# bbuchfink/diamond

Measured on AMD Instinct MI355X. Metric: GCUPS + aligned queries/s, blastp --fast, 10000 queries vs 1000000-seq DB (seed stage + banded SW extension), higher is better.
Workload: dtype int16

## Files before the change

### diamond_amd/csrc/seed_api.hip

```cpp
#include <hip/hip_runtime.h>
#include <algorithm>
#include <cstdlib>
#include <cmath>
#include <cstdio>
#include <cstring>
#include <string>
#include <sys/mman.h>
#include <thread>
#include <vector>
#include <chrono>
#include "ctx.h"
#include "seed_core.h"
#include "seed_kernels.h"

using namespace dmnd;

enum { SEED_CLASSES_LONG_DEFAULT = 1 };

static_assert(sizeof(dmnd_seed_params) == sizeof(SeedParams), "dmnd_seed_params must mirror dmnd::SeedParams");
static_assert(sizeof(dmnd_seed_hit) == 24, "dmnd_seed_hit layout");

extern "C" int dmnd_seed_params_fast(dmnd_seed_params* p, int threads)
{
	if (!p || threads < 1) return fail(DMND_E_ARG, "dmnd_seed_params_fast: bad argument");
// ... 281 lines not shown
			float ms = 0;
			if (hipEventElapsedTime(&ms, x.a, x.b) == hipSuccess) *x.into += ms;
			(void)hipEventDestroy(x.a); (void)hipEventDestroy(x.b);
		}
		spans.clear();
	}
};

}

struct SeedSizes {
	uint64_t slots, bm_words, bm1_words;
	uint32_t bm1_k3;
	int SB, slot_shift;
	bool fused, reuse;
	size_t bm_total;
};

static SeedSizes seed_sizes(const dmnd_ctx* c, const SeedParams& sp, int64_t nq_pos)
{
	SeedSizes z;
	const int S = sp.n_shapes;
	const uint64_t slots_x8 = (uint64_t)(tuning().seed_slots_x8 ? tuning().seed_slots_x8 : (seed_stream_can_fuse(sp) ? 32 : 16));
	z.slots = 1024;
	while (z.slots * 8 < (uint64_t)nq_pos * slots_x8) z.slots <<= 1;
	while (z.slots > ((uint64_t)1 << 31) && z.slots / 2 >= (uint64_t)nq_pos + (uint64_t)nq_pos / 4) z.slots >>= 1;

	uint64_t bm_words = 1 << 15;
	while (bm_words * 32 < (uint64_t)nq_pos * 16 && bm_words < ((uint64_t)1 << 22)) bm_words <<= 1;
	int bm1_log2 = 24;
	if (nq_pos > ((int64_t)1 << 24))
		while (bm1_log2 < 27 && ((uint64_t)1 << bm1_log2) < (uint64_t)nq_pos * 4) ++bm1_log2;
	uint64_t bm1_words = ((uint64_t)1 << bm1_log2) / 32;
	if (bm1_words > bm_words) bm1_words = bm_words;
	uint32_t bm1_k3 = 0;
	const bool long_seeds = !seed_stream_can_fuse(sp);
	if (long_seeds && bm1_log2 == 24 && bm_words >= 3 * bm1_words / 2) {
		bm1_words = 3 * bm1_words / 2;
		bm1_k3 = (uint64_t)nq_pos * 4 <= bm1_words * 32 ? 1u : 0u;
	}
	if (!long_seeds && bm1_log2 == 24 && bm_words >= 2 * bm1_words) { bm1_words *= 2; bm1_k3 = 1u; }
	bool fused = seed_stream_can_fuse(sp);
	if (const char* e = getenv("DMND_SEED_FUSED")) fused = fused && atoi(e) != 0;
	z.slot_shift = 4;
	const size_t set_bytes = (z.slots << z.slot_shift) + 2 * (size_t)nq_pos * sizeof(uint32_t) + (size_t)(bm_words + bm1_words) * sizeof(uint32_t);
	const bool reuse = c->reuse_query_index && set_bytes * (size_t)S <= ((size_t)64 << 30) && !getenv("DMND_SEED_MATCHED_CAP");
	const int SB = (fused && !reuse) ? 1 : S;
	const size_t bm_total = (size_t)SB * (bm_words + bm1_words) * sizeof(uint32_t);
	z.bm_words = bm_words; z.bm1_words = bm1_words; z.bm1_k3 = bm1_k3;
	z.fused = fused; z.reuse = reuse; z.SB = SB; z.bm_total = bm_total;
	return z;
}

static int seed_reserve(dmnd_ctx* c, const SeedParams& sp, const SeedSizes& z, int64_t nq_pos, int64_t q_end, int64_t q_block_len, bool generous)
{
	if (int rc = c->seed_bitmap.ensure(z.bm_total)) return rc;
	{
		const size_t held = c->qid_of.cap;
		if (int rc = c->qid_of.ensure((size_t)q_end * sizeof(uint32_t))) return rc;
		if (c->qid_of.cap != held) c->qid_of_version = ~(uint64_t)0;
	}
	if (int rc = c->mask_time.ensure((size_t)q_block_len + 256)) return rc;
	if (int rc = c->seed_keys.ensure((size_t)z.SB * (z.slots << z.slot_shift))) return rc;
	if (int rc = c->seed_need.ensure((size_t)(z.slots / 32 + SEED_NEED_FOLD_WORDS) * sizeof(uint32_t))) return rc;
	if (int rc = c->seed_next.ensure((size_t)seed_build_work_words(nq_pos) * sizeof(uint32_t))) return rc;
	if (int rc = c->seed_qlist.ensure((size_t)z.SB * nq_pos * sizeof(uint32_t))) return rc;
	if (int rc = c->seed_qkeys.ensure((size_t)nq_pos * sizeof(uint32_t))) return rc;
	if (!generous) return DMND_OK;
	const int64_t m_cap = std::max<int64_t>((int64_t)1 << 22, 4 * nq_pos);
	if (int rc = c->matched_slot.ensure((size_t)m_cap * sizeof(uint32_t))) return rc;
	if (int rc = c->matched_loc.ensure((size_t)m_cap * sizeof(int64_t))) return rc;
	if (int rc = c->seed_hits.ensure(((size_t)1 << 20) * sizeof(dmnd_seed_hit))) return rc;
	if (int rc = c->seed_deferred.ensure(((size_t)1 << 18) * sizeof(SeedDeferred))) return rc;
	if (z.fused) {
		if (int rc = c->seed_survivors.ensure(((size_t)1 << 20) * sizeof(SeedSurvivor))) return rc;
		if (int rc = c->seed_qfold.ensure((size_t)(q_block_len + 1) / 2 + 64)) return rc;
	}
	else {
		if (int rc = c->seed_survivors.ensure(((size_t)1 << 20) * sizeof(SeedSurvivor))) return rc;
		if (int rc = c->seed_scored.ensure(((size_t)1 << 20) * sizeof(SeedScored))) return rc;
	}
	return DMND_OK;
}

int dmnd_seed_query_ids(dmnd_ctx* c)
{
	const std::vector<int64_t>& ql = c->limits[DMND_QUERY];
	if (ql.size() < 2) return DMND_OK;
	const size_t bytes = (size_t)ql.back() * sizeof(uint32_t);
	if (c->qid_of_version == c->query_limits_version && c->qid_of.cap >= bytes) return DMND_OK;
	if (int rc = c->qid_of.ensure(bytes)) return rc;
	HIP_TRY(launch_seed_qid(c->d_limits[DMND_QUERY].as<int64_t>(), (int64_t)ql.size() - 1, c->qid_of.as<uint32_t>(), c->stream));
	c->qid_of_version = c->query_limits_version;
	return DMND_OK;
}

extern "C" int dmnd_seed_reserve(dmnd_ctx* c, const dmnd_seed_params* params, int64_t query_block_len)
{
	if (!c || !params || query_block_len <= 512) return fail(DMND_E_ARG, "dmnd_seed_reserve: bad argument");
	SeedParams sp;
	std::memcpy(&sp, params, sizeof(sp));
	if (sp.n_shapes < 1 || sp.n_shapes > SEED_MAX_SHAPES) return fail(DMND_E_ARG, "dmnd_seed_reserve: unsupported seed configuration");
	HIP_TRY(hipSetDevice(c->device));
	const int64_t nq_pos = query_block_len - 512;
	return seed_reserve(c, sp, seed_sizes(c, sp, nq_pos), nq_pos, query_block_len - 256, query_block_len, true);
}

namespace {

struct SeedHooks {
	bool trace;
	int chain, tiled, slices;
	int classes_long;
	uint64_t slices_budget;
	int64_t slices_min_letters;
	uint32_t slice_words;
	int64_t matched_cap, survivor_cap, hit_cap, deferred_cap;
	int64_t sort_cap, readback_bytes;
};
SeedHooks seed_hooks()
{
	auto num = [](const char* name, long long unset) { const char* e = getenv(name); return e ? atoll(e) : unset; };
	auto forced = [](const char* name) { const char* e = getenv(name); return e ? (atoi(e) != 0 ? 1 : 0) : -1; };
	auto cap = [](const char* name) { const char* e = getenv(name); return e ? std::max<int64_t>(1, atoll(e)) : (int64_t)0; };
	SeedHooks h;
	h.trace = getenv("DMND_TRACE") != nullptr;
	h.chain = forced("DMND_SEED_CHAIN"); h.tiled = forced("DMND_SEED_TILED"); h.slices = forced("DMND_SEED_SLICES");
	{ const char* e = getenv("DMND_SEED_CLASSES_LONG"); h.classes_long = e ? atoi(e) : -1; }
	h.slices_budget = (uint64_t)std::max<long long>(0, num("DMND_SEED_SLICES_BUDGET_MB", tuning().seed_slices_budget_mb)) << 20;
	h.slices_min_letters = num("DMND_SEED_SLICES_MIN_LETTERS", tuning().seed_slices_min_letters);
	h.slice_words = (uint32_t)std::min<long long>(SEED_SLICE_MAX_WORDS, std::max<long long>(64, num("DMND_SEED_SLICE_WORDS", SEED_SLICE_MAX_WORDS)));
	h.matched_cap = cap("DMND_SEED_MATCHED_CAP"); h.survivor_cap = cap("DMND_SEED_SURVIVOR_CAP");
	h.hit_cap = cap("DMND_SEED_HIT_CAP"); h.deferred_cap = cap("DMND_SEED_DEFERRED_CAP");
	const int64_t sort_cap = cap("DMND_SEED_SORT_CAP");
	h.sort_cap = std::min<int64_t>(sort_cap ? sort_cap : tuning().seed_sort_cap, (int64_t)1 << 24);
	h.readback_bytes = std::min<int64_t>(std::max<int64_t>(0, num("DMND_SEED_READBACK_BYTES", tuning().seed_readback_bytes)), (int64_t)1 << 30);
	return h;
}
int64_t cap_or(int64_t hook, int64_t computed) { return hook ? hook : computed; }

struct PostState {
	unsigned long long hits_seen = 0;
	bool hits_fresh = false;
	unsigned long long def_max = 0;
};
struct FusedHits { int64_t cap = 0, bound = 0; };

struct SeedRun {
	dmnd_ctx* c;
	SeedHooks hooks;
	SeedParams sp;
	hipStream_t st;
	int64_t q_begin = 0, q_end = 0, t_begin = 0, t_end = 0, nq_pos = 0, n_targets = 0;
	int S = 0;
	SeedSizes z;
	int slot_bits = 0, bm_log2 = 0;
	size_t slot_bytes = 0;
	bool nibble_shapes = true, classes_long = false;
	int classes = 0;
	bool mlr_on = false, lin_on = false, phases = false;
	bool index_ready = false;
	std::string signature;
	int64_t tiled_from = 0;
	SeedRefUse ref_use = SEED_REF_NONE;
	int slice_bits = -1;
	int64_t ref_windows = 0;
	std::vector<unsigned long long> counts;
	std::vector<int64_t> m_off;
	bool pristine = true;
	Timer tm;
	char path[128] = "host";
	unsigned long long n_pairs = 0;
	std::chrono::steady_clock::time_point lap_t0 = std::chrono::steady_clock::now();

	SeedRun(dmnd_ctx* ctx, const SeedHooks& h) : c(ctx), hooks(h), st(ctx->stream), tm(ctx->stream) {}
	int check_blocks();
	int geometry();
	int prepare();
	int ref_cache();
	int fused();
	int fused_stage2(SeedArgs a, int sid, unsigned long long n, unsigned long long ns, FusedHits& fh, PostState& ps);
	int after_post(const SeedArgs& a, int sid, int64_t n_matched, int64_t def_cap, PostState& ps);
	SeedArgs chain_args(const SeedChain& ch, int64_t def_cap, int sid) const;
	int chain(ChainResume& res);
	int phase1(const ChainResume& res);
	int count_pairs();
	int phase2(const ChainResume& res);
	int pair_filter(SeedArgs& a, int sid);
	int sort_hits();
	void trace_summary() const;

	void lap(const char* what) const
	{
		if (hooks.trace) std::fprintf(stderr, "dmnd_seed_search %8.2f ms  %s\n", std::chrono::duration<double, std::milli>(std::chrono::steady_clock::now() - lap_t0).count(), what);
	}
	unsigned long long* ctr() const { return c->counters.as<unsigned long long>(); }

	SeedArgs args_for(int sid, int64_t matched_cap, int64_t matched_off) const
	{
		const int own = sid % z.SB;
		SeedArgs a;
		a.params = sp;
		a.qdata = c->block[DMND_QUERY].as<int8_t>(); a.tdata = c->block[DMND_TARGET].as<int8_t>();
		a.qseed = c->soft_valid[DMND_QUERY] ? c->soft[DMND_QUERY].as<int8_t>() : a.qdata;
		a.tseed = (c->soft_valid[DMND_TARGET] && sp.seed_encoding == SEED_SPACED) ? c->soft[DMND_TARGET].as<int8_t>() : a.tdata;
		a.qlimits = c->d_limits[DMND_QUERY].as<int64_t>();
		a.q_begin = q_begin; a.q_end = q_end; a.t_begin = t_begin; a.t_end = t_end;
		a.qid_of = c->qid_of.as<uint32_t>(); a.mask_time = c->mask_time.as<uint8_t>();
		a.tlimits = c->d_limits[DMND_TARGET].as<int64_t>(); a.n_targets = n_targets;
		a.qwin = mlr_on ? c->seed_qwin.as<SeedQueryWindow>() : nullptr;
		a.lin_first = lin_on ? c->seed_lin_first.as<int64_t>() : nullptr;
		a.slots = reinterpret_cast<SeedSlot*>(c->seed_keys.as<char>() + (size_t)own * slot_bytes);
		a.slot_shift = z.slot_shift;
		a.qlist = c->seed_qlist.as<uint32_t>() + (size_t)own * nq_pos;
		a.slot_mask = z.slots - 1;
		a.classes = classes;
		a.slot_bits = slot_bits;
		a.bm1_hmask = bm1_hmask_of(slot_bits, classes);
		a.bitmap_log2 = bm_log2;
		a.phase_ticks = phases ? ctr() + S + 8 : nullptr;
		a.tclass = classes ? c->seed_tclass.as<uint16_t>() : nullptr; a.tclass_stride = (seed_code_groups(t_begin, t_end) + 3) & ~(int64_t)3;
		a.tcodes = classes ? c->seed_tcodes.as<uint64_t>() : nullptr; a.tflags = classes ? c->seed_tflags.as<uint32_t>() : nullptr; a.tplanes = classes ? c->seed_tplanes.as<uint64_t>() : nullptr;
		a.bitmap = c->seed_bitmap.as<uint32_t>() + (size_t)own * (z.bm_words + z.bm1_words);
		a.bitmap1 = a.bitmap + z.bm_words;
		a.bitmap1_words = (uint32_t)z.bm1_words; a.bitmap1_k3 = z.bm1_k3;
		a.matched_slot = c->matched_slot.as<uint32_t>() + matched_off;
		a.matched_loc = c->matched_loc.as<int64_t>() + matched_off;
		a.matched_count = ctr() + sid;
		a.matched_cap = matched_cap;
		a.deferred = nullptr; a.deferred_count = ctr() + S + 1; a.deferred_cap = 0;
// ... 43 lines not shown
		return fail(DMND_E_ARG, "dmnd_seed_search: unsupported seed configuration");
	if (sp.reduction_size > 20) return fail(DMND_E_ARG, "dmnd_seed_search: more than 20 reduced letter classes");
	for (int l = 0; l < 32; ++l)
		if (!((sp.reduction[l] >= 0 && sp.reduction[l] < sp.reduction_size) || sp.reduction[l] == L_MASK))
			return fail(DMND_E_ARG, "dmnd_seed_search: reduction map entry outside [0, reduction_size) and not the mask letter");
	for (int i = 0; i < sp.n_shapes; ++i) {
		if (sp.shape_len[i] < 1 || sp.shape_len[i] > 32 || sp.shape_weight[i] < 1 || sp.shape_weight[i] > 19 || sp.shape_weight[i] > sp.shape_len[i])
			return fail(DMND_E_ARG, "dmnd_seed_search: bad shape (length 1..32, weight 1..19)");
		uint32_t mask = 0;
		for (int k = 0; k < sp.shape_weight[i]; ++k) {
			if (sp.shape_pos[i][k] < 0 || sp.shape_pos[i][k] >= sp.shape_len[i]) return fail(DMND_E_ARG, "dmnd_seed_search: shape position outside the shape");
			mask |= 1u << sp.shape_pos[i][k];
		}
		if (mask != sp.shape_mask[i]) return fail(DMND_E_ARG, "dmnd_seed_search: shape mask and positions disagree");
	}
	if (sp.seed_encoding != SEED_SPACED && sp.seed_encoding != SEED_HASHED) return fail(DMND_E_ARG, "dmnd_seed_search: unknown seed encoding");
	if (sp.seed_encoding == SEED_HASHED) {
		if (sp.index_chunks != 1 || sp.reduction_size > 16) return fail(DMND_E_ARG, "dmnd_seed_search: the query-indexed mode runs with one index chunk and a 4-bit reduction");
		for (int i = 0; i < sp.n_shapes; ++i)
			if (sp.shape_len[i] > 16) return fail(DMND_E_ARG, "dmnd_seed_search: query-indexed mode with a shape longer than 16 letters");
	}
	return DMND_OK;
}

int SeedRun::check_blocks()
{
	const std::vector<int64_t>& ql = c->limits[DMND_QUERY];
	const std::vector<int64_t>& tl = c->limits[DMND_TARGET];
	mlr_on = c->min_length_ratio > 0.0;
	c->seed_qwin_n = 0;
	if (mlr_on) {
		if (c->query_contexts != 1 || sp.query_translated) return fail(DMND_E_ARG, "dmnd_seed_search: a minimum length ratio is not supported for translated searches");
		if (!lengths_non_increasing(ql.data(), (int64_t)ql.size() - 1)) return fail(DMND_E_ARG, "dmnd_seed_search: with a minimum length ratio the query block must be length-sorted (dmnd_length_sort_order)");
		if (!lengths_non_increasing(tl.data(), (int64_t)tl.size() - 1)) return fail(DMND_E_ARG, "dmnd_seed_search: with a minimum length ratio the reference block must be length-sorted (dmnd_length_sort_order)");
	}
	lin_on = c->linsearch;
	if (lin_on) {
		for (int i = 0; i < sp.n_shapes; ++i)
			if (!lin_shape_weight_ok(sp.shape_weight[i])) return fail(DMND_E_ARG, "dmnd_seed_search: Linearization is only supported for seed shapes of weight >= 10.");
		if (mlr_on) return fail(DMND_E_ARG, "dmnd_seed_search: the linearised search together with a minimum length ratio is not supported (dmnd_set_linsearch, dmnd_set_min_length_ratio)");
		if (c->lin_sorted_generation != c->target_generation) {
			if (!lengths_non_increasing(tl.data(), (int64_t)tl.size() - 1)) return fail(DMND_E_ARG, "dmnd_seed_search: the linearised search wants the reference block length-sorted (dmnd_length_sort_order)");
			c->lin_sorted_generation = c->target_generation;
		}
	}
	return DMND_OK;
}

int SeedRun::geometry()
{
	if (nq_pos >= 0xffffffffLL) return fail(DMND_E_ARG, "dmnd_seed_search: query block larger than 4G letters");
	S = sp.n_shapes;
	z = seed_sizes(c, sp, nq_pos);
	if (z.slots > ((uint64_t)1 << 31)) return fail(DMND_E_ARG, "dmnd_seed_search: query block too large for 32-bit slot numbers (more than 1.7 G seed positions): cut it into smaller blocks");
	slot_bytes = (size_t)z.slots << z.slot_shift;
	while (((uint64_t)1 << slot_bits) < z.slots) ++slot_bits;
	while (((uint64_t)1 << bm_log2) < z.bm_words) ++bm_log2;
	for (int i = 0; i < S; ++i) nibble_shapes = nibble_shapes && seed_nibble_mode(sp, i);
	classes_long = !z.fused && nibble_shapes && (hooks.classes_long >= 0 ? hooks.classes_long != 0 : SEED_CLASSES_LONG_DEFAULT && z.bm1_words * 32 >= ((uint64_t)1 << 25));
	classes = (z.fused || classes_long) && z.slots >= 64 && z.bm1_words % 8 == 0 && z.bm1_words >= 64 ? 8 : 0;
	if (z.fused && !classes) return fail(DMND_E_ARG, "dmnd_seed_search: fused seed search without key classes (table or level-1 filter too small for eighths)");
	if (z.reuse) {
		signature.assign(reinterpret_cast<const char*>(&sp), sizeof(sp));
		const uint64_t extra[7] = { c->query_generation, (uint64_t)nq_pos, z.slots, z.bm_words, z.bm1_words, (uint64_t)z.fused + 2 * (uint64_t)classes, (uint64_t)z.slot_shift * 2 + z.bm1_k3 };
		signature.append(reinterpret_cast<const char*>(extra), sizeof(extra));
	}
	index_ready = z.reuse && c->qindex_signature == signature && !signature.empty();
	c->qindex_signature.clear();
	tiled_from = hooks.tiled < 0 ? (int64_t)1 << 22 : hooks.tiled ? 0 : INT64_MAX;
	static const bool phases_on = getenv("DMND_SEED_PHASES") != nullptr;
	phases = phases_on;
	counts.assign((size_t)S + 1, 0); m_off.assign((size_t)S + 1, 0);
	lap("parameters checked");
	return DMND_OK;
}

int SeedRun::prepare()
{
	if (int rc = seed_reserve(c, sp, z, nq_pos, q_end, c->block_len[DMND_QUERY], false)) return rc;
	if (lin_on) {
		if (z.fused) return fail(DMND_E_ARG, "dmnd_seed_search: the linearised search has no form in the fused short-seed pipeline");
		if (int rc = c->seed_lin_first.ensure((size_t)z.slots * sizeof(int64_t))) return rc;
	}
	lap("buffers ensured");
	const bool counters_new = c->counters.cap < (size_t)chain_ctr_words(S) * sizeof(unsigned long long);
	if (int rc = c->counters.ensure((size_t)chain_ctr_words(S) * sizeof(unsigned long long))) return rc;
	{
		SeedClear clr;
		clr.add(c->counters.p, (size_t)((phases || counters_new) ? S + 16 : S + 8) * sizeof(unsigned long long), 0);
		clr.add(c->mask_time.p, (size_t)c->block_len[DMND_QUERY] + 256, SEED_NEVER);
		clr.add(c->seed_need.p, (size_t)(z.slots / 32) * sizeof(uint32_t), 0);
		if (!index_ready) {
			clr.add(c->seed_bitmap.p, z.bm_total, 0);
			clr.add(c->seed_keys.p, (size_t)z.SB * slot_bytes, 0xff);
		}
		HIP_TRY(launch_seed_clear(clr, st));
	}
	if (mlr_on) {
		if (int rc = c->seed_qwin.ensure((size_t)n_targets * sizeof(SeedQueryWindow))) return rc;
		HIP_TRY(launch_seed_qwin(c->d_limits[DMND_QUERY].as<int64_t>(), (int64_t)c->limits[DMND_QUERY].size() - 1, c->d_limits[DMND_TARGET].as<int64_t>(), n_targets, c->min_length_ratio, c->seed_qwin.as<SeedQueryWindow>(), st));
		c->seed_qwin_n = n_targets;
	}
	if (int rc = dmnd_seed_query_ids(c)) return rc;
	if (z.fused) {
		const int64_t nq = c->block_len[DMND_QUERY], nt = c->block_len[DMND_TARGET];
		if (int rc = c->seed_qfold.ensure((size_t)(nq + 1) / 2 + 64)) return rc;
		if (int rc = c->seed_tfold.ensure((size_t)(nt + 1) / 2 + 64)) return rc;
		HIP_TRY(launch_seed_fold(c->block[DMND_QUERY].as<int8_t>(), nq, c->seed_qfold.as<uint8_t>(), st));
		HIP_TRY(launch_seed_fold(c->block[DMND_TARGET].as<int8_t>(), nt, c->seed_tfold.as<uint8_t>(), st));
	}
	if (classes) {
		const int8_t* tseed = (c->soft_valid[DMND_TARGET] && sp.seed_encoding == SEED_SPACED) ? c->soft[DMND_TARGET].as<int8_t>() : c->block[DMND_TARGET].as<int8_t>();
		const int64_t n = seed_code_groups(t_begin, t_end);
		if (int rc = c->seed_tcodes.ensure((size_t)n * sizeof(uint64_t))) return rc;
		if (int rc = c->seed_tflags.ensure((size_t)n * sizeof(uint32_t))) return rc;
		if (int rc = c->seed_tplanes.ensure((size_t)n * sizeof(uint64_t))) return rc;
		if (int rc = c->seed_tclass.ensure((size_t)9 * (size_t)((n + 3) & ~(int64_t)3) * sizeof(uint16_t))) return rc;
		HIP_TRY(launch_seed_codes(sp, tseed, t_begin, t_end, c->seed_tcodes.as<uint64_t>(), c->seed_tflags.as<uint32_t>(), c->seed_tplanes.as<uint64_t>(), st));
	}
	for (int i = 0; i < 5; ++i) c->seed_ms[i] = 0;
	lap("clears and query ids enqueued");
	return DMND_OK;
}

int SeedRun::ref_cache()
{
	ref_windows = seed_ref_windows(t_begin, t_end);
	slice_bits = seed_slice_bits(z.bm1_words, slot_bits, hooks.slice_words);
	const bool sparse_filter = (uint64_t)nq_pos * 4 <= z.bm1_words * 32;
	const bool eligible = !z.fused && !classes && nibble_shapes && sp.seed_encoding == SEED_SPACED && slice_bits >= 0 && ref_windows < ((int64_t)1 << 31)
		&& (hooks.slices == 1 || (t_end - t_begin >= hooks.slices_min_letters && sparse_filter && c->seed_last_joined <= tuning().seed_slices_max_joined));
	const int8_t* tseed = c->soft_valid[DMND_TARGET] ? c->soft[DMND_TARGET].as<int8_t>() : c->block[DMND_TARGET].as<int8_t>();
	bool drop = false;
	ref_use = seed_ref_decide(c->seed_ref, seed_ref_key_of(c->target_generation, tseed, t_begin, t_end, sp, slice_bits), hooks.slices, eligible, seed_ref_cache_bytes(t_begin, t_end, S) + seed_ref_hash_bytes(t_begin, t_end, S), hooks.slices_budget, &drop);
	if (drop) c->release_seed_ref_buffers();
	if (ref_use != SEED_REF_BUILT) return DMND_OK;
	const int64_t n_groups = seed_code_groups(t_begin, t_end);
	DevBuf route[2];
	auto exact = [](DevBuf& b, size_t bytes) {
		if (b.cap == bytes && b.own) return true;
		b.release();
		if (hipMalloc(&b.p, bytes) != hipSuccess) { b.p = nullptr; (void)hipGetLastError(); return false; }
		b.cap = bytes;
		return true;
	};
	const bool ok = exact(c->seed_ref_codes, (size_t)n_groups * sizeof(uint64_t)) && c->seed_tflags.ensure((size_t)n_groups * sizeof(uint32_t)) == DMND_OK
		&& exact(c->seed_ref_lists, (size_t)S * (size_t)ref_windows * sizeof(uint32_t)) && exact(c->seed_ref_hashes, (size_t)S * (size_t)ref_windows * sizeof(uint32_t))
		&& exact(c->seed_ref_counts, (size_t)S * 64 * sizeof(uint32_t))
		&& exact(route[0], (size_t)ref_windows) && exact(route[1], (size_t)ref_windows);
	if (ok) {
		tm.start();
		hipError_t e = launch_seed_codes(sp, tseed, t_begin, t_end, c->seed_ref_codes.as<uint64_t>(), c->seed_tflags.as<uint32_t>(), nullptr, st);
		for (int sid = 0; sid < S && e == hipSuccess; ++sid) {
			uint32_t* list = c->seed_ref_lists.as<uint32_t>() + (size_t)sid * (size_t)ref_windows;
			e = launch_seed_route(sp, sid, c->seed_ref_codes.as<uint64_t>(), c->seed_tflags.as<uint32_t>(), t_begin, t_end, slice_bits, route[0].as<uint8_t>(), route[1].as<uint8_t>(),
				list, c->seed_ref_counts.as<uint32_t>() + (size_t)sid * 64, &c->sort_tmp, &c->sort_tmp_bytes, st);
			if (e == hipSuccess) e = launch_seed_ref_hashes(sp, sid, c->seed_ref_codes.as<uint64_t>(), list, t_begin, t_end, c->seed_ref_hashes.as<uint32_t>() + (size_t)sid * (size_t)ref_windows, st);
		}
		tm.stop(c->seed_ms[0]);
		if (e == hipSuccess) e = sync_stream(st);
		if (e != hipSuccess) { route[0].release(); route[1].release(); c->release_seed_ref(); HIP_TRY(e); }
	}
	route[0].release(); route[1].release();
	seed_ref_built(c->seed_ref, ok);
	if (!ok) { c->release_seed_ref(); ref_use = SEED_REF_NONE; }
	lap("reference cache built");
	return DMND_OK;
}

int seed_deferred_pass(dmnd_ctx* c, SeedArgs a, int sid, int64_t n_matched, int64_t nd, hipStream_t st)
{
	if (int rc = c->seed_eslot.ensure((size_t)n_matched * sizeof(uint64_t))) return rc;
	if (int rc = c->seed_eloc.ensure((size_t)n_matched * sizeof(uint64_t))) return rc;
	a.e_key = c->seed_eslot.as<uint64_t>();
	HIP_TRY(launch_seed_collect(a, n_matched, st));
	unsigned long long ne = 0;
	HIP_TRY(copy_now(st, &ne, a.e_count, sizeof(ne), hipMemcpyDeviceToHost));
	HIP_TRY(sort_keys_u64(c->seed_eslot.as<uint64_t>(), c->seed_eloc.as<uint64_t>(), (int64_t)ne, &c->sort_tmp, &c->sort_tmp_bytes, st));
	a.e_key = c->seed_eloc.as<uint64_t>();
	a.e_n = (int64_t)ne;
	HIP_TRY(launch_seed_deferred(a, sid, nd, st));
	return DMND_OK;
}

int SeedRun::after_post(const SeedArgs& a, int sid, int64_t n_matched, int64_t def_cap, PostState& ps)
{
	ps.hits_fresh = false;
	if (!sp.use_ungapped) return DMND_OK;
	unsigned long long both[2] = { 0, 0 };
	HIP_TRY(copy_now(st, both, a.hit_count, sizeof(both), hipMemcpyDeviceToHost));
	const unsigned long long nd = both[1];
	c->seed_trace[S + sid] = nd;
	if (nd == 0) { ps.hits_seen = both[0]; ps.hits_fresh = true; return DMND_OK; }
	ps.def_max = std::max(ps.def_max, nd);
	if ((int64_t)nd > def_cap) return DMND_OK;
	tm.start();
	if (int rc = seed_deferred_pass(c, a, sid, n_matched, (int64_t)nd, st)) return rc;
	tm.stop(c->seed_ms[3]);
	return DMND_OK;
}

int SeedRun::fused_stage2(SeedArgs a, int sid, unsigned long long n, unsigned long long ns, FusedHits& fh, PostState& ps)
{
	if (fh.bound + (int64_t)ns > fh.cap) {
		const int64_t new_cap = fh.bound + (int64_t)ns + (fh.bound + (int64_t)ns) / 2;
		DevBuf nb;
		if (int rc = nb.ensure((size_t)new_cap * sizeof(dmnd_seed_hit))) return rc;
		HIP_TRY(hipMemcpyAsync(nb.p, c->seed_hits.p, (size_t)fh.cap * sizeof(dmnd_seed_hit), hipMemcpyDeviceToDevice, st));
		HIP_TRY(sync_stream(st));
		c->seed_hits.release();
		c->seed_hits = nb;
		fh.cap = new_cap;
	}
	fh.bound += (int64_t)ns;
	if (int rc = c->seed_deferred.ensure((size_t)ns * sizeof(SeedDeferred))) return rc;
	a.hits = c->seed_hits.as<dmnd_seed_hit>(); a.hit_cap = fh.cap;
	a.deferred = c->seed_deferred.as<SeedDeferred>(); a.deferred_cap = (int64_t)ns;
	if (int rc = c->seed_scored.ensure((size_t)ns * sizeof(SeedScored))) return rc;
// ... 340 lines not shown

int SeedRun::sort_hits()
{
	const int64_t n = c->n_seed_hits;
	if (n > 0xffffffffLL) return fail(DMND_E_CAP, "dmnd_seed_search: more than 2^32 seed hits in one block pair");
	if (int rc = c->seed_hits_sorted.ensure((size_t)n * sizeof(dmnd_seed_hit))) return rc;
	if (int rc = c->sort_keys[0].ensure((size_t)n * sizeof(uint64_t))) return rc;
	if (int rc = c->sort_keys[1].ensure((size_t)n * sizeof(uint64_t))) return rc;
	if (int rc = c->sort_idx[0].ensure((size_t)n * sizeof(uint32_t))) return rc;
	if (int rc = c->sort_idx[1].ensure((size_t)n * sizeof(uint32_t))) return rc;
	uint64_t* keys[2] = { c->sort_keys[0].as<uint64_t>(), c->sort_keys[1].as<uint64_t>() };
	uint32_t* idx[2] = { c->sort_idx[0].as<uint32_t>(), c->sort_idx[1].as<uint32_t>() };
	const HitSortBits bits = hit_sort_bits(c);
	HIP_TRY(sort_seed_hits(c->seed_hits.as<dmnd_seed_hit>(), c->seed_hits_sorted.as<dmnd_seed_hit>(), n, keys, idx, &c->sort_tmp, &c->sort_tmp_bytes, st,
		bits.query, bits.subject, bits.off, !sp.use_ungapped));
	HIP_TRY(sync_stream(st));
	return DMND_OK;
}

void SeedRun::trace_summary() const
{
	std::fprintf(stderr, "dmnd_seed_search: %d shapes, %lld query positions, joined reference positions per shape:", S, (long long)nq_pos);
	for (int sid = 0; sid < S; ++sid) std::fprintf(stderr, " %llu", counts[sid]);
	std::fprintf(stderr, " | pairs %llu | Hamming survivors:", n_pairs);
	for (int sid = 0; sid < S && (size_t)sid < c->seed_trace.size(); ++sid) std::fprintf(stderr, " %llu", c->seed_trace[sid]);
	std::fprintf(stderr, " | deferred:");
	for (int sid = 0; sid < S && (size_t)(S + sid) < c->seed_trace.size(); ++sid) std::fprintf(stderr, " %llu", c->seed_trace[S + sid]);
	std::fprintf(stderr, " | hits %lld | ms index %.2f stream %.2f mask %.2f pairs %.2f | path: %s\n", (long long)c->n_seed_hits, c->seed_ms[0], c->seed_ms[1], c->seed_ms[2], c->seed_ms[3], path);
	const size_t held = c->seed_ref_codes.cap + c->seed_ref_lists.cap + c->seed_ref_hashes.cap + c->seed_ref_counts.cap;
	if (ref_use == SEED_REF_NONE) std::fprintf(stderr, "dmnd_seed_search: stream: plain, reference cache: none, %zu bytes held\n", held);
	else std::fprintf(stderr, "dmnd_seed_search: stream: slices (%d x %g KB), reference cache: %s, %zu bytes held\n", 1 << slice_bits, (double)(z.bm1_words >> slice_bits) * 4 / 1024, ref_use == SEED_REF_BUILT ? "built" : "kept", held);
}

}

extern "C" int dmnd_seed_search(dmnd_ctx* c, const dmnd_seed_params* params, int64_t* n_hits)
{
	if (!c || !params || !n_hits) return fail(DMND_E_ARG, "dmnd_seed_search: NULL argument");
	SeedRun r(c, seed_hooks());
	*n_hits = 0;
	c->n_seed_hits = 0;
	c->seed_ret_hits = -1;
	const std::vector<int64_t>& ql = c->limits[DMND_QUERY];
	const std::vector<int64_t>& tl = c->limits[DMND_TARGET];
	if (ql.size() < 2 || tl.size() < 2) return fail(DMND_E_ARG, "dmnd_seed_search: both blocks must be uploaded with limits");
	std::memcpy(&r.sp, params, sizeof(r.sp));
	if (int rc = seed_check_params(r.sp)) return rc;
	if (int rc = r.check_blocks()) return rc;
	HIP_TRY(hipSetDevice(c->device));
	r.q_begin = ql.front(); r.q_end = ql.back(); r.t_begin = tl.front(); r.t_end = tl.back();
	r.nq_pos = r.q_end - r.q_begin; r.n_targets = (int64_t)tl.size() - 1;
	if (r.nq_pos <= 0 || r.t_end <= r.t_begin) return DMND_OK;
	if (int rc = r.geometry()) return rc;
	if (int rc = r.prepare()) return rc;
	if (int rc = r.ref_cache()) return rc;
	if (c->soft_valid[DMND_QUERY]) HIP_TRY(launch_seed_soft_time(r.args_for(0, 0, 0), r.st));
	ChainResume res;
	if (r.z.fused) {
		if (int rc = r.fused()) return rc;
	}
	else {
		res.cap_total = cap_or(r.hooks.matched_cap, std::max<int64_t>(std::max<int64_t>((int64_t)1 << 22, 4 * r.nq_pos), (int64_t)std::min(c->matched_loc.cap / sizeof(int64_t), c->matched_slot.cap / sizeof(uint32_t))));
		if (r.hooks.chain >= 0 ? r.hooks.chain != 0 : chain_by_default(c, r.classes_long))
			if (int rc = r.chain(res)) return rc;
		if (res.phase1_again)
			if (int rc = r.phase1(res)) return rc;
		if (r.hooks.trace)
			if (int rc = r.count_pairs()) return rc;
		r.lap("phase 1 done (index, stream, mask of every shape)");
		if (!res.hits_done)
			if (int rc = r.phase2(res)) return rc;
	}
	r.lap("filters done");
	if (r.z.reuse) c->qindex_signature = r.signature;
	if (c->n_seed_hits > 0 && !res.hits_done)
		if (int rc = r.sort_hits()) return rc;
	r.lap("hits sorted");
	if (r.phases) {
		unsigned long long t[8];
		HIP_TRY(copy_now(r.st, t, r.ctr() + r.S + 8, sizeof(t), hipMemcpyDeviceToHost));
		std::fprintf(stderr, "SEED_PHASES (ms of workgroup time, summed): start %.1f | windows %.1f | level 1 %.1f | table %.1f | light lists %.1f | heavy lists %.1f\n",
			t[0] / 1e5, t[1] / 1e5, t[2] / 1e5, t[3] / 1e5, t[4] / 1e5, t[5] / 1e5);
	}
	r.tm.collect();
	c->seed_ms[4] = c->seed_ms[0] + c->seed_ms[1] + c->seed_ms[2] + c->seed_ms[3];
	if (r.hooks.trace) r.trace_summary();
	*n_hits = c->n_seed_hits;
	c->seed_last_hits = c->n_seed_hits;
	c->seed_last_joined = 0;
	for (int sid = 0; sid < r.S; ++sid) c->seed_last_joined += (int64_t)r.counts[sid];
	return DMND_OK;
}

extern "C" int64_t dmnd_seed_hit_count(const dmnd_ctx* c) { return c ? c->n_seed_hits : -1; }

extern "C" int dmnd_set_seed_hits_resident(dmnd_ctx* c, int on)
{
	if (!c) return fail(DMND_E_ARG, "dmnd_set_seed_hits_resident: ctx is NULL");
	c->seed_hits_stay = on != 0;
	return DMND_OK;
}

extern "C" int dmnd_seed_hits(dmnd_ctx* c, dmnd_seed_hit* out, int64_t cap)
{
	if (!c || (!out && c->n_seed_hits > 0)) return fail(DMND_E_ARG, "dmnd_seed_hits: NULL argument");
	if (cap < c->n_seed_hits) return fail(DMND_E_CAP, "dmnd_seed_hits: buffer too small");
// ... 10 lines not shown
```

### diamond_amd/csrc/seed_core.h

```cpp
#pragma once
#include <stdint.h>
#include "swipe_core.h"

namespace dmnd {

enum { SEED_MAX_SHAPES = 64, SEED_MAX_WEIGHT = 32, L_MASK = 23, L_STOP = 24, L_DELIM = 31, SEED_NEVER = 255 };
enum { SEED_SPACED = 0, SEED_HASHED = 1 };

struct SeedParams {
	int32_t n_shapes;
	int32_t shape_len[SEED_MAX_SHAPES], shape_weight[SEED_MAX_SHAPES];
	uint32_t shape_mask[SEED_MAX_SHAPES];
	int8_t shape_pos[SEED_MAX_SHAPES][SEED_MAX_WEIGHT];
	int8_t reduction[32];
	int32_t reduction_size;
	int32_t seedp_bits, index_chunks, hamming_filter_id;
	int32_t ungapped_window, left_most_interval;
	double seed_complexity_cut;
	int32_t use_ungapped, short_query_max_len, short_query_cutoff;
	int32_t cutoff_table[32];
	int32_t tile_size, simd_lanes;
	int32_t query_translated;
	int32_t seed_encoding;
	int32_t cutoff_table_short[32];
// ... 314 lines not shown
		if (!admit((int64_t)(locs[k] & LOC))) continue;
		if (fingerprint_id(q, tdata + (int64_t)(locs[k] & LOC)) < c.hamming_filter_id) continue;
		++L; r += k < rank;
	}
	const int64_t lanes = c.simd_lanes, left = L - r / lanes * lanes;
	return (int)(left < lanes ? left : lanes);
}
struct SeedAdmitAll { DMND_HD bool operator()(int64_t) const { return true; } };
DMND_HD int simd_batch_size_sorted(const SeedParams& c, const uint64_t* locs, int64_t n, const int8_t* tdata, const int8_t* q, int64_t sloc)
{
	return simd_batch_size_sorted(c, locs, n, tdata, q, sloc, SeedAdmitAll());
}

DMND_HD uint32_t seed_hash_a(uint64_t x)
{
	const uint32_t lo = (uint32_t)x, hi = (uint32_t)(x >> 32);
	uint32_t a = lo * 0x9E3779B1u + hi * 0x85EBCA6Bu;
	a ^= a >> 15; a *= 0x2C1B3C6Du; a ^= a >> 13;
	return a;
}

DMND_HD uint32_t seed_hash_b(uint64_t x)
{
	const uint32_t lo = (uint32_t)x, hi = (uint32_t)(x >> 32);
	uint32_t b = (lo ^ 0x68E31DA4u) * 0xCC9E2D51u + (hi + 0x1B873593u) * 0x27D4EB2Fu;
	b ^= b >> 16; b *= 0x85EBCA6Bu; b ^= b >> 13;
	return b;
}

DMND_HD uint64_t seed_hash(uint64_t x) { return ((uint64_t)seed_hash_b(x) << 32) | seed_hash_a(x); }

DMND_HD uint32_t bm1_word(uint32_t h, uint32_t words) { return (uint32_t)(((uint64_t)h * words) >> 32); }
DMND_HD uint32_t seed_class(uint64_t key)
{
	uint32_t x = (uint32_t)key ^ (uint32_t)(key >> 32);
	x ^= x >> 16;
	x ^= x >> 8;
	x ^= x >> 4;
	return (x ^ (x >> 3)) & 7u;
}
DMND_HD uint32_t seed_order(uint32_t h, uint64_t key, int classes) { return classes ? seed_class(key) << 29 | h >> 3 : h; }
DMND_HD uint32_t bm1_hmask_of(int slot_bits, int classes) { return ~0u << (32 - slot_bits + (classes ? 3 : 0)); }
DMND_HD uint32_t bm1_word_of_top(uint32_t t, int slot_bits, uint32_t words) { return bm1_word(t << (32 - slot_bits), words); }
DMND_HD uint32_t bm1_word_of_key(uint32_t h, uint64_t key, int classes, uint32_t hmask, uint32_t words)
{
	if (!classes) return bm1_word(h & hmask, words);
	const uint32_t w8 = words >> 3;
	return seed_class(key) * w8 + bm1_word(h & hmask, w8);
}
DMND_HD uint32_t bm2_word_of_top(uint32_t t, int slot_bits, int bm_log2) { return (uint32_t)(((uint64_t)t << bm_log2) >> slot_bits); }
DMND_HD uint32_t bm1_bits(uint32_t h, uint32_t k3)
{
	const uint32_t two = (1u << (h & 31)) | (1u << ((h >> 5) & 31));
	return k3 ? two | (1u << ((h >> 10) & 31)) : two;
}

}
```

### diamond_amd/csrc/seed_kernels.hip

```cpp
#include <hip/hip_runtime.h>
#include <stdint.h>
#include "seed_core.h"
#include <algorithm>
#include <cstdlib>
#include <cstring>
#include <cstdio>
#include <rocprim/device/device_radix_sort.hpp>
#include <rocprim/iterator/counting_iterator.hpp>
#include <rocprim/iterator/transform_iterator.hpp>
#include <rocprim/iterator/transform_output_iterator.hpp>
#include <rocprim/device/device_scan.hpp>
#include "seed_kernels.h"

namespace dmnd {

struct SeedClearArgs { char* p[8]; uint64_t bytes[8]; uint64_t first_chunk[9]; uint32_t word[8]; int n; };
__global__ __launch_bounds__(256) void seed_clear_kernel(SeedClearArgs z)
{
	const uint64_t t = (uint64_t)blockIdx.x * blockDim.x + threadIdx.x;
	if (t >= z.first_chunk[8]) return;
	char* base = z.p[0];
	uint64_t bytes = z.bytes[0], first = 0;
	uint32_t w = z.word[0];
#pragma unroll
// ... 737 lines not shown
	const unsigned wave = threadIdx.x >> 6, lane = threadIdx.x & 63u;
	unsigned qn = 0, sn = 0;
	auto rank_in = [&](unsigned long long ballot) { return (unsigned)__builtin_amdgcn_mbcnt_hi((uint32_t)(ballot >> 32), __builtin_amdgcn_mbcnt_lo((uint32_t)ballot, 0u)); };
	auto wave_sync = [&]() { __builtin_amdgcn_fence(__ATOMIC_RELEASE, "wavefront"); __builtin_amdgcn_wave_barrier(); __builtin_amdgcn_fence(__ATOMIC_ACQUIRE, "wavefront"); };
	auto flush = [&]() {
		const unsigned n = sn < ST ? sn : ST;
		unsigned long long at = 0;
		if (lane == 0) at = atomicAdd(a.matched_count, (unsigned long long)n);
		at = ((unsigned long long)(uint32_t)__shfl((int)(at >> 32), 0) << 32) | (uint32_t)__shfl((int)(uint32_t)at, 0);
		wave_sync();
		if (lane < n && at + lane < (unsigned long long)a.matched_cap) { a.matched_slot[at + lane] = st_slot[wave][lane]; a.matched_loc[at + lane] = base + st_off[wave][lane]; }
		wave_sync();
		sn = 0;
	};
	auto probe = [&](bool active, uint64_t seed, uint32_t off) {
		bool found = false;
		uint64_t slot = 0;
		if (active) {
			const uint64_t hh = seed_hash(seed);
			if (!a.level2 || ((a.bitmap[a.bm2_index((uint32_t)hh, seed)] >> (uint32_t)(hh >> 59)) & 1u)) {
				slot = a.home(hh, seed);
				SeedSlot sl = a.slot(slot);
				uint32_t fl = 0;
				for (;;) {
					if (sl.key == SEED_EMPTY) break;
					if (sl.key == seed) { found = true; fl = sl.flags; break; }
					slot = (slot + 1) & a.slot_mask;
					sl = a.slot(slot);
				}
				if (found && !(fl & SLOT_JOINED)) a.slot(slot).flags = fl | SLOT_JOINED;
			}
		}
		const unsigned long long jb = __ballot(found);
		if (jb == 0) return;
		const unsigned k = sn + rank_in(jb);
		if (found) {
			if (k < ST) { st_slot[wave][k] = (uint32_t)slot; st_off[wave][k] = off; }
			else {
				const unsigned long long idx = atomicAdd(a.matched_count, 1ull);
				if (idx < (unsigned long long)a.matched_cap) { a.matched_slot[idx] = (uint32_t)slot; a.matched_loc[idx] = base + off; }
			}
		}
		sn += (unsigned)__builtin_popcountll(jb);
		if (sn >= ST / 2) flush();
	};
	auto probe_queued = [&](bool active, uint32_t e) {
		const uint32_t off = active ? e : 0u;
		const uint64_t seed = seed_window_key(codes[off >> 4], codes[(off >> 4) + 1], off & 15u, care64);
		probe(active, seed, off);
	};
	typedef uint32_t u32x4 __attribute__((ext_vector_type(4)));
	static_assert(B == 4, "one 16-byte load per round");
	const uint64_t stride = (uint64_t)B * blockDim.x, first = (lo & ~(uint64_t)(B - 1)) + (uint64_t)B * threadIdx.x;
	u32x4 hv[DEPTH], ov[DEPTH];
	auto request = [&](uint64_t k, u32x4& h, u32x4& o) {
		h = 0; o = 0;
		if (k < hi) {
			h = __builtin_nontemporal_load(reinterpret_cast<const u32x4*>(hashes + k));
			o = __builtin_nontemporal_load(reinterpret_cast<const u32x4*>(list + k));
		}
	};
#pragma unroll
	for (int d = 0; d < DEPTH; ++d) request(first + (uint64_t)d * stride, hv[d], ov[d]);
	for (uint64_t k0 = first; k0 < hi + (uint64_t)B * threadIdx.x; k0 += (uint64_t)DEPTH * stride) {
#pragma unroll
		for (int d = 0; d < DEPTH; ++d) {
			const u32x4 h4 = hv[d], o4 = ov[d];
			const uint64_t k = k0 + (uint64_t)d * stride;
			request(k + (uint64_t)DEPTH * stride, hv[d], ov[d]);
#pragma unroll
			for (int j = 0; j < B; ++j) {
				const uint32_t h = h4[j];
				const uint32_t lw = seed_slice_word(h, a.bm1_hmask, a.bitmap1_words) - word0;
				const uint32_t bw = slice[lw < slice_words ? lw : 0u], need = bm1_bits(h, a.bitmap1_k3);
				const bool pass = k + j >= lo && k + j < hi && (bw & need) == need;
				const unsigned long long pb = __ballot(pass);
				if (pb) {
					if (pass) q_off[wave][qn + rank_in(pb)] = o4[j];
					qn += (unsigned)__builtin_popcountll(pb);
					if (qn >= 64) {
						wave_sync();
						qn -= 64;
						const uint32_t e = q_off[wave][qn + lane];
						wave_sync();
						probe_queued(true, e);
					}
				}
			}
		}
	}
	wave_sync();
	probe_queued(lane < qn, lane < qn ? q_off[wave][lane] : 0u);
	if (sn) flush();
}

__global__ __launch_bounds__(256) void seed_route_kernel(const uint64_t* __restrict__ codes, const uint32_t* __restrict__ flags, int64_t base, int64_t n_groups, int64_t t_begin, int64_t t_end,
	int len, uint32_t care, uint64_t care64, int slice_bits, uint8_t* __restrict__ route, uint32_t* __restrict__ counts)
{
	__shared__ uint32_t hist[1 << SEED_SLICE_MAX_BITS];
	if (threadIdx.x < (1u << SEED_SLICE_MAX_BITS)) hist[threadIdx.x] = 0;
	__syncthreads();
	const int64_t g = (int64_t)blockIdx.x * blockDim.x + threadIdx.x;
	if (g < n_groups) {
		const int64_t p0 = base + 16 * g;
		uint8_t out[16];
		seed_route_group(codes[g], codes[g + 1], flags[g], flags[g + 1], t_begin - p0, t_end - p0, len, care, care64, slice_bits, out);
		uint32_t w[4] = { 0, 0, 0, 0 };
#pragma unroll
		for (int j = 0; j < 16; ++j) {
			w[j >> 2] |= (uint32_t)out[j] << ((j & 3) * 8);
			if (out[j] != SEED_ROUTE_NONE) atomicAdd(&hist[out[j]], 1u);
		}
		typedef uint32_t u32x4 __attribute__((ext_vector_type(4)));
		u32x4 v; v.x = w[0]; v.y = w[1]; v.z = w[2]; v.w = w[3];
		*reinterpret_cast<u32x4*>(route + 16 * g) = v;
	}
	__syncthreads();
	if (threadIdx.x < (1u << slice_bits) && hist[threadIdx.x]) atomicAdd(&counts[threadIdx.x], hist[threadIdx.x]);
}

__global__ void seed_mask_kernel(SeedArgs a, int sid)
{
	const uint64_t slot = (uint64_t)blockIdx.x * blockDim.x + threadIdx.x;
	if (slot > a.slot_mask) return;
	const SeedSlot sl = a.slot(slot);
	if (sl.key == SEED_EMPTY || !(sl.flags & SLOT_JOINED)) return;
	const uint32_t count = sl.flags >> 8;
	if (a.fused ? !(sl.flags & SLOT_LOWC) : seed_is_complex(a.params, sid, a.qdata + a.q_begin + (count == 1 ? sl.head : a.qlist[sl.head]))) return;
	a.slot(slot).flags = sl.flags | SLOT_ERASED;
	const int t = sid * a.params.index_chunks + seed_chunk(a.params, seed_of_key(a.params, sid, sl.key));
	for (uint32_t i = 0; i < count; ++i) {
		const uint32_t x = count == 1 ? sl.head : a.qlist[sl.head + i];
		const uint8_t old = a.mask_time[a.q_begin + x];
		if (t < old) a.mask_time[a.q_begin + x] = (uint8_t)t;
	}
}

template<bool CHAIN>
__global__ void seed_mask_joined_kernel(SeedArgs a, int sid, int64_t n_matched, SeedChain ch)
{
	int64_t m = (int64_t)blockIdx.x * blockDim.x + threadIdx.x, end = n_matched;
	if (CHAIN) {
		if (ch.ctr[chain_ctr_status(ch.S)] & CHAIN_MATCHED_OVER) return;
		m += sid ? (int64_t)ch.ctr[sid - 1] : 0;
		end = (int64_t)ch.ctr[sid];
// ... 1300 lines not shown
```

### diamond_amd/csrc/seed_slices_core.h

```cpp
#pragma once
#include <stdint.h>
#include <string.h>
#include "seed_core.h"
#include "seed_ref_state.h"

namespace dmnd {

enum { SEED_SLICE_MAX_WORDS = 32768, SEED_SLICE_MAX_BITS = 6 };
enum : uint8_t { SEED_ROUTE_NONE = 0xff };

DMND_HD int seed_slice_bits(uint64_t words, int slot_bits, uint32_t max_words)
{
	if (max_words > (uint32_t)SEED_SLICE_MAX_WORDS) max_words = SEED_SLICE_MAX_WORDS;
	for (int b = 0; b <= SEED_SLICE_MAX_BITS; ++b) {
		if (words == 0 || words % ((uint64_t)1 << b) != 0) return -1;
		if ((words >> b) <= max_words) return b <= slot_bits ? b : -1;
	}
	return -1;
}

DMND_HD uint32_t seed_slice_of(uint32_t h, int slice_bits) { return slice_bits ? h >> (32 - slice_bits) : 0u; }

DMND_HD uint32_t seed_slice_word(uint32_t h, uint32_t hmask, uint32_t words) { return bm1_word(h & hmask, words); }
DMND_HD uint64_t seed_window_key(uint64_t c0, uint64_t c1, uint32_t at, uint64_t care64)
{
	const int sh = 4 * (int)at;
	return (sh == 0 ? c0 : (c0 >> sh) | (c1 << (64 - sh))) & care64;
}
DMND_HD uint32_t seed_ref_hash_entry(const uint64_t* codes, uint32_t off, uint64_t care64)
{
	return seed_hash_a(seed_window_key(codes[off >> 4], codes[(off >> 4) + 1], off & 15u, care64));
}

DMND_HD void seed_route_group(uint64_t c0, uint64_t c1, uint32_t f0, uint32_t f1, int64_t first, int64_t last, int len, uint32_t care, uint64_t care64, int slice_bits, uint8_t out[16])
{
	const uint32_t delim = (f0 & 0xffffu) | (f1 << 16), bad = (f0 >> 16) | (f1 & 0xffff0000u);
	const uint32_t span = (1u << len) - 1;
	for (int w = 0; w < 16; ++w) {
		const bool inside = w >= first && w < last && ((delim >> w) & span) == 0;
		const bool ok = inside && ((bad >> w) & care) == 0;
		const uint64_t key = seed_window_key(c0, c1, (uint32_t)w, care64);
		out[w] = ok ? (uint8_t)seed_slice_of(seed_hash_a(key), slice_bits) : (uint8_t)SEED_ROUTE_NONE;
	}
}

struct SeedRefKey {
	uint64_t generation;
	const void* tseed;
	int64_t t_begin, t_end;
	int32_t n_shapes, slice_bits, seed_encoding, reduction_size;
	int8_t reduction[32];
	int32_t shape_len[SEED_MAX_SHAPES];
	uint32_t shape_mask[SEED_MAX_SHAPES];
};

inline SeedRefKey seed_ref_key_of(uint64_t generation, const void* tseed, int64_t t_begin, int64_t t_end, const SeedParams& sp, int slice_bits)
{
	SeedRefKey k;
	memset(&k, 0, sizeof(k));
	k.generation = generation; k.tseed = tseed; k.t_begin = t_begin; k.t_end = t_end;
	k.n_shapes = sp.n_shapes; k.slice_bits = slice_bits; k.seed_encoding = sp.seed_encoding; k.reduction_size = sp.reduction_size;
	memcpy(k.reduction, sp.reduction, sizeof(k.reduction));
	for (int i = 0; i < sp.n_shapes && i < SEED_MAX_SHAPES; ++i) { k.shape_len[i] = sp.shape_len[i]; k.shape_mask[i] = sp.shape_mask[i]; }
	return k;
}

inline std::string seed_ref_key_bytes(const SeedRefKey& k) { return std::string(reinterpret_cast<const char*>(&k), sizeof(SeedRefKey)); }

inline int64_t seed_ref_windows(int64_t t_begin, int64_t t_end) { return ((t_end - (t_begin & ~(int64_t)15) + 15) / 16) * 16; }
inline uint64_t seed_ref_cache_bytes(int64_t t_begin, int64_t t_end, int n_shapes)
{
// ... 27 lines not shown
```

Before: 218.0.

## Enlarge level-1 filter for sliced reference path and defer list loads past filter

When the reference-slice cache is used, the level-1 query bitmap filter is resized to the largest power-of-two that fits the slice geometry and gets a third hash bit via a new k3 mode, aiming to reject more reference windows before probing. The decision about the reference cache now runs before buffer reservation so the bitmap can be sized for the sliced layout, with a fallback that restores the plain sizes and clears the bitmap if the cache build fails. In the probe kernel, the offset list is no longer streamed alongside the hashes; only passing positions are queued and their list entries are fetched afterwards. This cuts bandwidth for filtered-out windows but adds a dependent gather for survivors and uses more bitmap memory.

```diff
diff --git a/diamond_amd/csrc/seed_api.hip b/diamond_amd/csrc/seed_api.hip
--- a/diamond_amd/csrc/seed_api.hip
+++ b/diamond_amd/csrc/seed_api.hip
@@ -357,9 +357,20 @@
 	return z;
 }
 
-static int seed_reserve(dmnd_ctx* c, const SeedParams& sp, const SeedSizes& z, int64_t nq_pos, int64_t q_end, int64_t q_block_len, bool generous)
-{
-	if (int rc = c->seed_bitmap.ensure(z.bm_total)) return rc;
+static SeedSizes seed_sizes_sliced(const dmnd_ctx* c, const SeedParams& sp, int64_t nq_pos, const SeedSizes& z, uint32_t slice_words, uint64_t forced_words)
+{
+	if (z.fused || seed_stream_can_fuse(sp) || sp.seed_encoding != SEED_SPACED || nq_pos > ((int64_t)1 << 24) || c->reuse_query_index) return z;
+	int slot_bits = 0;
+	while (((uint64_t)1 << slot_bits) < z.slots) ++slot_bits;
+	SeedSizes s = z;
+	s.bm1_words = seed_slices_filter_words((uint64_t)nq_pos, slot_bits, z.bm_words, z.bm1_words, slice_words, forced_words, &s.bm1_k3);
+	s.bm_total = (size_t)s.SB * (s.bm_words + s.bm1_words) * sizeof(uint32_t);
+	return s;
+}
+
+static int seed_reserve(dmnd_ctx* c, const SeedParams& sp, const SeedSizes& z, size_t bitmap_bytes, int64_t nq_pos, int64_t q_end, int64_t q_block_len, bool generous)
+{
+	if (int rc = c->seed_bitmap.ensure(std::max(z.bm_total, bitmap_bytes))) return rc;
 	{
 		const size_t held = c->qid_of.cap;
 		if (int rc = c->qid_of.ensure((size_t)q_end * sizeof(uint32_t))) return rc;
@@ -408,7 +419,8 @@
 	if (sp.n_shapes < 1 || sp.n_shapes > SEED_MAX_SHAPES) return fail(DMND_E_ARG, "dmnd_seed_reserve: unsupported seed configuration");
 	HIP_TRY(hipSetDevice(c->device));
 	const int64_t nq_pos = query_block_len - 512;
-	return seed_reserve(c, sp, seed_sizes(c, sp, nq_pos), nq_pos, query_block_len - 256, query_block_len, true);
+	const SeedSizes z = seed_sizes(c, sp, nq_pos);
+	return seed_reserve(c, sp, z, seed_sizes_sliced(c, sp, nq_pos, z, SEED_SLICE_MAX_WORDS, 0).bm_total, nq_pos, query_block_len - 256, query_block_len, true);
 }
 
 namespace {
@@ -420,6 +432,8 @@
 	uint64_t slices_budget;
 	int64_t slices_min_letters;
 	uint32_t slice_words;
+	bool slices_alloc_fail;
+	uint64_t slices_filter_words;
 	int64_t matched_cap, survivor_cap, hit_cap, deferred_cap;
 	int64_t sort_cap, readback_bytes;
 };
@@ -435,6 +449,8 @@
 	h.slices_budget = (uint64_t)std::max<long long>(0, num("DMND_SEED_SLICES_BUDGET_MB", tuning().seed_slices_budget_mb)) << 20;
 	h.slices_min_letters = num("DMND_SEED_SLICES_MIN_LETTERS", tuning().seed_slices_min_letters);
 	h.slice_words = (uint32_t)std::min<long long>(SEED_SLICE_MAX_WORDS, std::max<long long>(64, num("DMND_SEED_SLICE_WORDS", SEED_SLICE_MAX_WORDS)));
+	h.slices_alloc_fail = forced("DMND_SEED_SLICES_ALLOC_FAIL") == 1;
+	h.slices_filter_words = (uint64_t)std::max<long long>(0, num("DMND_SEED_SLICES_FILTER_WORDS", 0));
 	h.matched_cap = cap("DMND_SEED_MATCHED_CAP"); h.survivor_cap = cap("DMND_SEED_SURVIVOR_CAP");
 	h.hit_cap = cap("DMND_SEED_HIT_CAP"); h.deferred_cap = cap("DMND_SEED_DEFERRED_CAP");
 	const int64_t sort_cap = cap("DMND_SEED_SORT_CAP");
@@ -458,7 +474,7 @@
 	hipStream_t st;
 	int64_t q_begin = 0, q_end = 0, t_begin = 0, t_end = 0, nq_pos = 0, n_targets = 0;
 	int S = 0;
-	SeedSizes z;
+	SeedSizes z, z_sliced;
 	int slot_bits = 0, bm_log2 = 0;
 	size_t slot_bytes = 0;
 	bool nibble_shapes = true, classes_long = false;
@@ -481,6 +497,7 @@
 	SeedRun(dmnd_ctx* ctx, const SeedHooks& h) : c(ctx), hooks(h), st(ctx->stream), tm(ctx->stream) {}
 	int check_blocks();
 	int geometry();
+	void ref_decide();
 	int prepare();
 	int ref_cache();
 	int fused();
@@ -630,6 +647,7 @@
 	if (nq_pos >= 0xffffffffLL) return fail(DMND_E_ARG, "dmnd_seed_search: query block larger than 4G letters");
 	S = sp.n_shapes;
 	z = seed_sizes(c, sp, nq_pos);
+	z_sliced = seed_sizes_sliced(c, sp, nq_pos, z, hooks.slice_words, hooks.slices_filter_words);
 	if (z.slots > ((uint64_t)1 << 31)) return fail(DMND_E_ARG, "dmnd_seed_search: query block too large for 32-bit slot numbers (more than 1.7 G seed positions): cut it into smaller blocks");
 	slot_bytes = (size_t)z.slots << z.slot_shift;
 	while (((uint64_t)1 << slot_bits) < z.slots) ++slot_bits;
@@ -640,7 +658,7 @@
 	if (z.fused && !classes) return fail(DMND_E_ARG, "dmnd_seed_search: fused seed search without key classes (table or level-1 filter too small for eighths)");
 	if (z.reuse) {
 		signature.assign(reinterpret_cast<const char*>(&sp), sizeof(sp));
-		const uint64_t extra[7] = { c->query_generation, (uint64_t)nq_pos, z.slots, z.bm_words, z.bm1_words, (uint64_t)z.fused + 2 * (uint64_t)classes, (uint64_t)z.slot_shift * 2 + z.bm1_k3 };
+		const uint64_t extra[7] = { c->query_generation, (uint64_t)nq_pos, z.slots, z.bm_words, z.bm1_words, (uint64_t)z.fused + 2 * (uint64_t)classes, (uint64_t)z.slot_shift * 4 + z.bm1_k3 };
 		signature.append(reinterpret_cast<const char*>(extra), sizeof(extra));
 	}
 	index_ready = z.reuse && c->qindex_signature == signature && !signature.empty();
@@ -655,7 +673,7 @@
 
 int SeedRun::prepare()
 {
-	if (int rc = seed_reserve(c, sp, z, nq_pos, q_end, c->block_len[DMND_QUERY], false)) return rc;
+	if (int rc = seed_reserve(c, sp, z, z_sliced.bm_total, nq_pos, q_end, c->block_len[DMND_QUERY], false)) return rc;
 	if (lin_on) {
 		if (z.fused) return fail(DMND_E_ARG, "dmnd_seed_search: the linearised search has no form in the fused short-seed pipeline");
 		if (int rc = c->seed_lin_first.ensure((size_t)z.slots * sizeof(int64_t))) return rc;
@@ -701,10 +719,10 @@
 	return DMND_OK;
 }
 
-int SeedRun::ref_cache()
+void SeedRun::ref_decide()
 {
 	ref_windows = seed_ref_windows(t_begin, t_end);
-	slice_bits = seed_slice_bits(z.bm1_words, slot_bits, hooks.slice_words);
+	slice_bits = seed_slice_bits(z_sliced.bm1_words, slot_bits, hooks.slice_words);
 	const bool sparse_filter = (uint64_t)nq_pos * 4 <= z.bm1_words * 32;
 	const bool eligible = !z.fused && !classes && nibble_shapes && sp.seed_encoding == SEED_SPACED && slice_bits >= 0 && ref_windows < ((int64_t)1 << 31)
 		&& (hooks.slices == 1 || (t_end - t_begin >= hooks.slices_min_letters && sparse_filter && c->seed_last_joined <= tuning().seed_slices_max_joined));
@@ -712,7 +730,13 @@
 	bool drop = false;
 	ref_use = seed_ref_decide(c->seed_ref, seed_ref_key_of(c->target_generation, tseed, t_begin, t_end, sp, slice_bits), hooks.slices, eligible, seed_ref_cache_bytes(t_begin, t_end, S) + seed_ref_hash_bytes(t_begin, t_end, S), hooks.slices_budget, &drop);
 	if (drop) c->release_seed_ref_buffers();
+	if (ref_use != SEED_REF_NONE) z = z_sliced;
+}
+
+int SeedRun::ref_cache()
+{
 	if (ref_use != SEED_REF_BUILT) return DMND_OK;
+	const int8_t* tseed = c->soft_valid[DMND_TARGET] ? c->soft[DMND_TARGET].as<int8_t>() : c->block[DMND_TARGET].as<int8_t>();
 	const int64_t n_groups = seed_code_groups(t_begin, t_end);
 	DevBuf route[2];
 	auto exact = [](DevBuf& b, size_t bytes) {
@@ -722,7 +746,7 @@
 		b.cap = bytes;
 		return true;
 	};
-	const bool ok = exact(c->seed_ref_codes, (size_t)n_groups * sizeof(uint64_t)) && c->seed_tflags.ensure((size_t)n_groups * sizeof(uint32_t)) == DMND_OK
+	const bool ok = !hooks.slices_alloc_fail && exact(c->seed_ref_codes, (size_t)n_groups * sizeof(uint64_t)) && c->seed_tflags.ensure((size_t)n_groups * sizeof(uint32_t)) == DMND_OK
 		&& exact(c->seed_ref_lists, (size_t)S * (size_t)ref_windows * sizeof(uint32_t)) && exact(c->seed_ref_hashes, (size_t)S * (size_t)ref_windows * sizeof(uint32_t))
 		&& exact(c->seed_ref_counts, (size_t)S * 64 * sizeof(uint32_t))
 		&& exact(route[0], (size_t)ref_windows) && exact(route[1], (size_t)ref_windows);
@@ -741,7 +765,17 @@
 	}
 	route[0].release(); route[1].release();
 	seed_ref_built(c->seed_ref, ok);
-	if (!ok) { c->release_seed_ref(); ref_use = SEED_REF_NONE; }
+	if (!ok) {
+		c->release_seed_ref(); ref_use = SEED_REF_NONE;
+		const SeedSizes plain = seed_sizes(c, sp, nq_pos);
+		const bool moved = plain.bm1_words != z.bm1_words || plain.bm1_k3 != z.bm1_k3;
+		z = plain;
+		if (moved && !index_ready) {
+			SeedClear clr;
+			clr.add(c->seed_bitmap.p, z.bm_total, 0);
+			HIP_TRY(launch_seed_clear(clr, st));
+		}
+	}
 	lap("reference cache built");
 	return DMND_OK;
 }
@@ -1188,6 +1222,7 @@
 	r.nq_pos = r.q_end - r.q_begin; r.n_targets = (int64_t)tl.size() - 1;
 	if (r.nq_pos <= 0 || r.t_end <= r.t_begin) return DMND_OK;
 	if (int rc = r.geometry()) return rc;
+	r.ref_decide();
 	if (int rc = r.prepare()) return rc;
 	if (int rc = r.ref_cache()) return rc;
 	if (c->soft_valid[DMND_QUERY]) HIP_TRY(launch_seed_soft_time(r.args_for(0, 0, 0), r.st));
diff --git a/diamond_amd/csrc/seed_core.h b/diamond_amd/csrc/seed_core.h
--- a/diamond_amd/csrc/seed_core.h
+++ b/diamond_amd/csrc/seed_core.h
@@ -390,6 +390,7 @@
 DMND_HD uint32_t bm1_bits(uint32_t h, uint32_t k3)
 {
 	const uint32_t two = (1u << (h & 31)) | (1u << ((h >> 5) & 31));
+	if (k3 == 2) return two | (1u << (((h & 0x7ffu) * 0x9E3779B1u) >> 27));
 	return k3 ? two | (1u << ((h >> 10) & 31)) : two;
 }
 
diff --git a/diamond_amd/csrc/seed_kernels.hip b/diamond_amd/csrc/seed_kernels.hip
--- a/diamond_amd/csrc/seed_kernels.hip
+++ b/diamond_amd/csrc/seed_kernels.hip
@@ -813,22 +813,19 @@
 	typedef uint32_t u32x4 __attribute__((ext_vector_type(4)));
 	static_assert(B == 4, "one 16-byte load per round");
 	const uint64_t stride = (uint64_t)B * blockDim.x, first = (lo & ~(uint64_t)(B - 1)) + (uint64_t)B * threadIdx.x;
-	u32x4 hv[DEPTH], ov[DEPTH];
-	auto request = [&](uint64_t k, u32x4& h, u32x4& o) {
-		h = 0; o = 0;
-		if (k < hi) {
-			h = __builtin_nontemporal_load(reinterpret_cast<const u32x4*>(hashes + k));
-			o = __builtin_nontemporal_load(reinterpret_cast<const u32x4*>(list + k));
-		}
+	u32x4 hv[DEPTH];
+	auto request = [&](uint64_t k, u32x4& h) {
+		h = 0;
+		if (k < hi) h = __builtin_nontemporal_load(reinterpret_cast<const u32x4*>(hashes + k));
 	};
 #pragma unroll
-	for (int d = 0; d < DEPTH; ++d) request(first + (uint64_t)d * stride, hv[d], ov[d]);
+	for (int d = 0; d < DEPTH; ++d) request(first + (uint64_t)d * stride, hv[d]);
 	for (uint64_t k0 = first; k0 < hi + (uint64_t)B * threadIdx.x; k0 += (uint64_t)DEPTH * stride) {
 #pragma unroll
 		for (int d = 0; d < DEPTH; ++d) {
-			const u32x4 h4 = hv[d], o4 = ov[d];
+			const u32x4 h4 = hv[d];
 			const uint64_t k = k0 + (uint64_t)d * stride;
-			request(k + (uint64_t)DEPTH * stride, hv[d], ov[d]);
+			request(k + (uint64_t)DEPTH * stride, hv[d]);
 #pragma unroll
 			for (int j = 0; j < B; ++j) {
 				const uint32_t h = h4[j];
@@ -837,21 +834,21 @@
 				const bool pass = k + j >= lo && k + j < hi && (bw & need) == need;
 				const unsigned long long pb = __ballot(pass);
 				if (pb) {
-					if (pass) q_off[wave][qn + rank_in(pb)] = o4[j];
+					if (pass) q_off[wave][qn + rank_in(pb)] = (uint32_t)(k + j);
 					qn += (unsigned)__builtin_popcountll(pb);
 					if (qn >= 64) {
 						wave_sync();
 						qn -= 64;
-						const uint32_t e = q_off[wave][qn + lane];
+						const uint32_t at = q_off[wave][qn + lane];
 						wave_sync();
-						probe_queued(true, e);
+						probe_queued(true, list[at]);
 					}
 				}
 			}
 		}
 	}
 	wave_sync();
-	probe_queued(lane < qn, lane < qn ? q_off[wave][lane] : 0u);
+	probe_queued(lane < qn, lane < qn ? list[q_off[wave][lane]] : 0u);
 	if (sn) flush();
 }
 
diff --git a/diamond_amd/csrc/seed_slices_core.h b/diamond_amd/csrc/seed_slices_core.h
--- a/diamond_amd/csrc/seed_slices_core.h
+++ b/diamond_amd/csrc/seed_slices_core.h
@@ -17,6 +17,20 @@
 		if ((words >> b) <= max_words) return b <= slot_bits ? b : -1;
 	}
 	return -1;
+}
+
+DMND_HD uint64_t seed_slices_filter_words(uint64_t nq_pos, int slot_bits, uint64_t bm_words, uint64_t default_words, uint32_t max_slice_words, uint64_t forced_words, uint32_t* k3)
+{
+	uint64_t w = forced_words;
+	if (w == 0) {
+		uint64_t most = (uint64_t)SEED_SLICE_MAX_WORDS << SEED_SLICE_MAX_BITS;
+		if (bm_words < most) most = bm_words;
+		for (w = 1; w * 2 <= most; w *= 2) {}
+		if (w <= default_words) return default_words;
+	}
+	if (w == default_words || seed_slice_bits(w, slot_bits, max_slice_words) < 0) return default_words;
+	if (k3) *k3 = nq_pos * 4 > w * 32 ? 0u : (w & (w - 1)) == 0 ? 2u : 1u;
+	return w;
 }
 
 DMND_HD uint32_t seed_slice_of(uint32_t h, int slice_bits) { return slice_bits ? h >> (32 - slice_bits) : 0u; }
```

New measurement: 250.8, median of 6. +15.0%, better.
